# CognitiveAISystems/MAPF-GPT

Hardware: AMD Instinct MI355X
Metric: agent-steps/s (env+obs+GPT fwd) (higher is better)
Workload: dtype f16x3

## Files before the change

mapf_gpt_amd/csrc/gpt_kernels_c256b.h:

```cpp
#pragma once
#include "gpt_kernels_c256p.h"
#include "gpt_kernels_attn_tiles.h"

namespace mgpt {
namespace fastk {

constexpr int kA256oProjSteps = 16;
constexpr int kA256oPeriod = 8 * kA256StepsPerHead + kA256oProjSteps;


template <class T, int NP>
__global__ __launch_bounds__(256) void pack_attn256q_kernel(const float *__restrict__ w_attn, const float *__restrict__ gain,
                                                            const float *__restrict__ w_proj, uint16_t *__restrict__ out,
                                                            float scale_a, float scale_p)
{
    constexpr int C = 256, NH = 8, QKV = NH * kA256StepsPerHead;
    const int64_t gid = (int64_t)blockIdx.x * 256 + threadIdx.x;
    if (gid >= (int64_t)kA256oPeriod * 8 * 64) return;
    const int lane = (int)(gid & 63), ms = (int)((gid >> 6) & 7), G = (int)(gid >> 9);
    const int rho = lane & 15, qk = lane >> 4;
    float v[8];
    if (G < QKV) {
        const int head = G / kA256StepsPerHead, st = G - head * kA256StepsPerHead;
        int which, kb, dim;
        if (st < 4) {
            const int cc = 4 * st + (ms >> 1), ug = ms & 1, rq = rho >> 2;
            kb = cc >> 1; which = cc & 1;
            const int blk = which == 0 ? 2 * (rq & 1) + (rq >> 1) : rq;
            dim = 8 * blk + 4 * ug + (rho & 3);
        } else { which = 2; kb = 4 * (st - 4) + (ms >> 1); dim = 16 * (ms & 1) + rho; }
        const float *row = w_attn + (size_t)(which * C + head * 32 + dim) * C;
#pragma unroll
        for (int e = 0; e < 8; e++) {
            const int col = 32 * kb + 8 * qk + e;
            v[e] = row[col] * gain[col] * scale_a;
        }
    } else {
        const int s = G - QKV, tt = s >> 2, j = s & 3;
        const int cc = 4 * j + (ms >> 1), kb = cc >> 1, fgl = 2 * (cc & 1) + (ms & 1);
        const float *row = w_proj + (size_t)(64 * tt + 16 * fgl + rho) * C;
#pragma unroll
        for (int e = 0; e < 8; e++) {
            const int col = 32 * kb + (e & 3) + 8 * (2 * (qk & 1) + (e >> 2)) + 4 * (qk >> 1);
            v[e] = row[col] * scale_p;
        }
    }
    u32x2 h0, l0, h1, l1;
    split4<T, NP>(v, h0, l0);
    split4<T, NP>(v + 4, h1, l1);
    u32x4 hi, lo;
    hi[0] = h0[0]; hi[1] = h0[1]; hi[2] = h1[0]; hi[3] = h1[1];
    lo[0] = l0[0]; lo[1] = l0[1]; lo[2] = l1[0]; lo[3] = l1[1];
    uint16_t *dst = out + (((size_t)G * 8 + ms) * NP) * 512 + (size_t)lane * 8;
    *reinterpret_cast<u32x4 *>(dst) = hi;
    if (NP == 2) *reinterpret_cast<u32x4 *>(dst + 512) = lo;
}

template <int NP> constexpr int kL0TabHeadBytes = 192 * NP;
template <int NP> constexpr int kL0TabEntryBytes = 8 * kL0TabHeadBytes<NP>;
template <class T, int NP, int STAMPS = 0, bool EMB = false, int TAB = 0>
__global__ __launch_bounds__(512, 2) void attn256q_kernel(float *__restrict__ x, const uint16_t *__restrict__ wstream, float inv_scale,
                                                          float scale_log2e, float inv_proj, unsigned char *__restrict__ spill,
                                                          int n_rows, unsigned long long *stamps = nullptr,
                                                          const unsigned char *__restrict__ tokens = nullptr, const float *__restrict__ etab = nullptr,
                                                          unsigned char *__restrict__ table = nullptr)
{
    static_assert(TAB == 0 || (TAB == 1 && EMB) || (TAB == 2 && !EMB && STAMPS == 0), "table modes");
    constexpr int HB = kL0TabHeadBytes<NP>, ENT = kL0TabEntryBytes<NP>;
    constexpr int C = 256, KS = 16, NH = 8, HS = 32, NW = 8;
    static_assert(NP == 2 || NP == 1, "planes");
    constexpr int MS = 8;
    constexpr int STEP = MS * NP * 1024;
    constexpr int NSLOT = 5;
    constexpr int PW = MS * NP / NW;
    constexpr int KROW = 80, VROW = 528;
    constexpr int NSPILL = 2 * NP;
    constexpr int NYLD = 14 * NP;
    static_assert(PW >= 1, "a wave moves at least one piece per step");
    extern __shared__ __attribute__((aligned(16))) unsigned char smem[];
    const int tid = threadIdx.x, lane = tid & 63;
    const int wave = __builtin_amdgcn_readfirstlane(tid >> 6);
    const int tok0 = wave * 32;
    const unsigned lane16 = (unsigned)lane * 16u;
    const unsigned lds0 = (unsigned)(size_t)smem + lane16;
    const unsigned sK = (unsigned)(size_t)smem + NSLOT * STEP, sV = sK + NP * kT * KROW;
    constexpr int PERIOD = TAB == 2 ? kA256oProjSteps : kA256oPeriod;
    const unsigned char *wbase = reinterpret_cast<const unsigned char *>(wstream) + (size_t)(wave * PW) * 1024 +
                                 (TAB == 2 ? (size_t)(kA256oPeriod - kA256oProjSteps) * STEP : 0);
    unsigned char *sp_wave = spill + ((size_t)blockIdx.x * NW + wave) * (size_t)(14 * NP * 1024);
    const int n_mine = n_rows > (int)blockIdx.x ? (n_rows - 1 - (int)blockIdx.x) / (int)gridDim.x + 1 : 0;
    unsigned long long ts[8] = {0, 0, 0, 0, 0, 0, 0, 0}, t_mark = 0;
    auto phase = [&](int i) {
        if constexpr (STAMPS == 1 || STAMPS == 3) { const unsigned long long t = __builtin_readcyclecounter(); ts[i] += t - t_mark; t_mark = t; }
    };
    auto smark = [&]() { if constexpr (STAMPS == 2) t_mark = __builtin_readcyclecounter(); };
    auto sphase = [&](int i) {
        if constexpr (STAMPS == 2) { const unsigned long long t = __builtin_readcyclecounter(); ts[i] += t - t_mark; t_mark = t; }
    };
    if constexpr (STAMPS != 0) { ts[0] = __builtin_readcyclecounter(); ts[1] = wall_clock64(); t_mark = ts[0]; }
    if (n_mine == 0) return;

    int r_issue = 0;
    int slot_cur = 0, slot_prev = NSLOT - 1;
    unsigned cur_addr = 0, nxt_addr = 0;
    auto issue = [&](int slot) {
        const unsigned char *src = wbase + (size_t)r_issue * STEP;
        unsigned char *dst = smem + (size_t)slot * STEP + (size_t)(wave * PW) * 1024;
#pragma unroll
        for (int i = 0; i < PW; i++) dma_piece(src + lane16, dst, std::integral_constant<int, 0>{}, i);
        r_issue = r_issue + 1 == PERIOD ? 0 : r_issue + 1;
    };
#pragma unroll
    for (int G = 0; G < NSLOT - 1; G++) issue(G);
    auto sync_wait = [&](auto pending_c) {
        vm_wait<decltype(pending_c)::value>();
        __builtin_amdgcn_s_barrier();
    };
    int slot_refill = 0;
    auto sync_issue = [&]() {
        issue(slot_prev);
        const int slot_next = slot_cur + 1 == NSLOT ? 0 : slot_cur + 1;
        cur_addr = lds0 + (unsigned)slot_cur * STEP;
        nxt_addr = lds0 + (unsigned)slot_next * STEP;
        slot_prev = slot_cur;
        slot_cur = slot_next;
    };
    u32x4 wb[2][2][2];
    auto lds_frag = [&](unsigned addr, auto off_c, u32x4 &dst) {
        asm volatile("ds_read_b128 %0, %1 offset:%2" : "=v"(dst) : "v"(addr), "n"(decltype(off_c)::value) : "memory");
    };
    auto lds_pair = [&](unsigned slot_addr, auto ms_c, u32x4 (&dst)[2]) {
        constexpr int ms = decltype(ms_c)::value;
        lds_frag(slot_addr, std::integral_constant<int, ms * NP * 1024>{}, dst[0]);
        if (NP == 2) lds_frag(slot_addr, std::integral_constant<int, (ms * NP + 1) * 1024>{}, dst[1]);
        else dst[1] = dst[0];
    };
    auto chunk_begin = [&](auto c_c, auto next_c) {
        constexpr int c = decltype(c_c)::value;
        asm volatile("s_waitcnt lgkmcnt(0)" ::: "memory");
        __builtin_amdgcn_sched_barrier(0);
        if (c < 3) { lds_pair(cur_addr, std::integral_constant<int, 2 * c + 2>{}, wb[(c + 1) & 1][0]); lds_pair(cur_addr, std::integral_constant<int, 2 * c + 3>{}, wb[(c + 1) & 1][1]); }
        else if (decltype(next_c)::value) { lds_pair(nxt_addr, std::integral_constant<int, 0>{}, wb[0][0]); lds_pair(nxt_addr, std::integral_constant<int, 1>{}, wb[0][1]); }
        __builtin_amdgcn_sched_barrier(0);
    };
    constexpr bool PLACED = true;
    auto chunk_wait = [&]() {
        asm volatile("s_waitcnt lgkmcnt(0)" ::: "memory");
        __builtin_amdgcn_sched_barrier(0);
    };
    auto chunk_read = [&](auto c_c, auto next_c, auto n_c) {
        constexpr int c = decltype(c_c)::value, n = decltype(n_c)::value;
        if constexpr (n < 2 * NP) {
            constexpr int fr = n / NP, pl = n % NP;
            if constexpr (c < 3) lds_frag(cur_addr, std::integral_constant<int, ((2 * c + 2 + fr) * NP + pl) * 1024>{}, wb[(c + 1) & 1][fr][pl]);
            else if constexpr (decltype(next_c)::value) lds_frag(nxt_addr, std::integral_constant<int, (fr * NP + pl) * 1024>{}, wb[0][fr][pl]);
            if constexpr (NP == 1 && (c < 3 || decltype(next_c)::value)) wb[(c + 1) & 1][fr][1] = wb[(c + 1) & 1][fr][0];
            __builtin_amdgcn_sched_barrier(0);
        }
    };
    auto pin6 = [&]() {
#pragma unroll
        for (int n = 0; n < (NP == 2 ? 12 : 4); n++) __builtin_amdgcn_sched_group_barrier(0x008, 1, 0);
        __builtin_amdgcn_sched_barrier(0);
    };
    auto pack_octet = [&](const f32x16 &v, int m, u32x4 (&dst)[2]) {
#pragma unroll
        for (int wd = 0; wd < 4; wd++) {
            unsigned a, b2;
            split2p<T, NP>(v[8 * m + 2 * wd], v[8 * m + 2 * wd + 1], a, b2);
            dst[0][wd] = a; dst[1][wd] = b2;
        }
    };
    auto mm16 = [&](const u32x4 &a, const u32x4 &b2, f32x16 &blk, auto s_c) {
        constexpr int S = decltype(s_c)::value;
        f32x4 c = {blk[4 * S], blk[4 * S + 1], blk[4 * S + 2], blk[4 * S + 3]};
        c = T::mfma16(a, b2, c);
        blk[4 * S] = c[0]; blk[4 * S + 1] = c[1]; blk[4 * S + 2] = c[2]; blk[4 * S + 3] = c[3];
    };
    auto mm16z = [&](const u32x4 &a, const u32x4 &b2, f32x16 &blk, auto s_c) {
        constexpr int S = decltype(s_c)::value;
        f32x4 c = {0.f, 0.f, 0.f, 0.f};
        c = T::mfma16(a, b2, c);
        blk[4 * S] = c[0]; blk[4 * S + 1] = c[1]; blk[4 * S + 2] = c[2]; blk[4 * S + 3] = c[3];
    };
    using I0 = std::integral_constant<int, 0>;
    using I1 = std::integral_constant<int, 1>;
    using I2 = std::integral_constant<int, 2>;
    using I3 = std::integral_constant<int, 3>;
    auto mma4 = [&](const u32x4 (&w0)[2], const u32x4 (&w1)[2], const u32x4 (&x0)[2], const u32x4 (&x1)[2], f32x16 &blk, auto swap_c, auto first_c, auto &&behind) {
        constexpr bool SW = decltype(swap_c)::value, FIRST = decltype(first_c)::value;
        auto one = [&](const u32x4 &w, const u32x4 &xx, auto s_c) {
            if constexpr (SW) mm16(xx, w, blk, s_c); else mm16(w, xx, blk, s_c);
        };
        auto onez = [&](const u32x4 &w, const u32x4 &xx, auto s_c) {
            if constexpr (!FIRST) one(w, xx, s_c);
            else if constexpr (SW) mm16z(xx, w, blk, s_c);
            else mm16z(w, xx, blk, s_c);
        };
        if (NP == 2) {
            onez(w0[1], x0[0], I0{}); behind(I0{}); onez(w1[1], x0[0], I1{}); behind(I1{}); onez(w0[1], x1[0], I2{}); behind(I2{}); onez(w1[1], x1[0], I3{}); behind(I3{});
            one(w0[0], x0[1], I0{}); behind(std::integral_constant<int, 4>{}); one(w1[0], x0[1], I1{}); behind(std::integral_constant<int, 5>{});
            one(w0[0], x1[1], I2{}); one(w1[0], x1[1], I3{});
            one(w0[0], x0[0], I0{}); one(w1[0], x0[0], I1{}); one(w0[0], x1[0], I2{}); one(w1[0], x1[0], I3{});
        } else {
            onez(w0[0], x0[0], I0{}); behind(I0{}); onez(w1[0], x0[0], I1{}); behind(I1{}); onez(w0[0], x1[0], I2{}); behind(I2{}); onez(w1[0], x1[0], I3{});
        }
    };
    auto chunk_body = [&](auto c_c, auto next_c, auto &&mm) {
        if constexpr (PLACED) {
            chunk_wait();
            constexpr bool REFILL = false;
            constexpr int N_REFILL = NP == 2 ? 5 : 2, N_LAST = REFILL ? N_REFILL : 2 * NP - 1, NMF = NP == 2 ? 12 : 4;
            mm([&](auto n_c) {
                constexpr int n = decltype(n_c)::value;
                if constexpr (n < 2 * NP) { __builtin_amdgcn_sched_barrier(0); chunk_read(c_c, next_c, n_c); }
                else if constexpr (REFILL && n == N_REFILL) { __builtin_amdgcn_sched_barrier(0); issue(slot_refill); __builtin_amdgcn_sched_barrier(0); }
            });
#pragma unroll
            for (int n = 0; n < NMF - 1 - N_LAST; n++) __builtin_amdgcn_sched_group_barrier(0x008, 1, 0);
            __builtin_amdgcn_sched_barrier(0);
        } else {
            chunk_begin(c_c, next_c);
            mm([&](auto) {});
            pin6();
        }
    };
    auto fold4 = [&](float v) {
        float a = v, b2 = v;
        asm volatile("s_nop 1\n\tv_permlane16_swap_b32 %0, %1" : "+v"(a), "+v"(b2));
        float c = a + b2, d = c;
        asm volatile("s_nop 1\n\tv_permlane32_swap_b32 %0, %1" : "+v"(c), "+v"(d));
        return c + d;
    };
    auto row_swap = [&](unsigned &a, unsigned &b2) {
        asm volatile("s_nop 1\n\tv_permlane16_swap_b32 %0, %1" : "+v"(a), "+v"(b2));
    };
    auto half_swap = [&](float v, float &lower, float &upper) {
        lower = v; upper = v;
        asm volatile("s_nop 1\n\tv_permlane32_swap_b32 %0, %1" : "+v"(lower), "+v"(upper));
    };
    auto other_half_max = [&](float v) { float a, b2; half_swap(v, a, b2); return fmaxf(a, b2); };
    auto other_half_sum = [&](float v) { float a, b2; half_swap(v, a, b2); return a + b2; };
    constexpr bool QK_UNITS = true;
    const float sc2 = 1.0f;
    const float q_units = scale_log2e * inv_scale, k_units = inv_scale;

    u32x4 xn[KS][2];

    f32x16 qa, ka;
    auto step_pair = [&](auto j_c, auto pending_c, auto &&after_barrier, auto next_c) {
        constexpr int j = decltype(j_c)::value;
        smark();
        sync_wait(pending_c);
        after_barrier();
        sync_issue();
        sphase(2);
        auto chunk = [&](auto c_c) {
            constexpr int c = decltype(c_c)::value;
            constexpr int cc = 4 * j + c, kb = cc >> 1;
            chunk_body(c_c, next_c, [&](auto &&behind) {
                using F = std::integral_constant<bool, (cc < 2)>;
                if constexpr ((cc & 1) == 0) mma4(wb[c & 1][0], wb[c & 1][1], xn[kb], xn[8 + kb], qa, std::false_type{}, F{}, behind);
                else mma4(wb[c & 1][0], wb[c & 1][1], xn[kb], xn[8 + kb], ka, std::false_type{}, F{}, behind);
            });
            asm volatile("" : "+v"(qa), "+v"(ka));
        };
        chunk(I0{}); chunk(I1{}); chunk(I2{}); chunk(I3{});
        sphase(4);
    };
    auto nothing = [&]() {};
    asm volatile("s_waitcnt vmcnt(0)" ::: "memory");
    __builtin_amdgcn_s_barrier();
    nxt_addr = lds0;
    using P4 = std::integral_constant<int, PW * (NSLOT - 3)>;
    using P4S = std::integral_constant<int, PW * (NSLOT - 3) + NSPILL>;

#pragma unroll 1
    for (int k = 0; k < n_mine; k++) {
        const int64_t b = (int64_t)blockIdx.x + (int64_t)k * gridDim.x;
        unsigned char *xw = reinterpret_cast<unsigned char *>(x + (b * kT + tok0) * C);
        unsigned ent0 = 0, ent1 = 0;
        if constexpr (TAB == 2) {
            unsigned l16p = lane16;
            asm volatile("" : "+v"(l16p));
            const unsigned char *tk = tokens + b * kT + tok0;
            const unsigned tt_p = (l16p >> 4) & 15u;
            unsigned id0, id1;
            asm volatile("global_load_ubyte %0, %1, %2" : "=v"(id0) : "v"(tt_p), "s"(tk) : "memory");
            asm volatile("global_load_ubyte %0, %1, %2 offset:16" : "=v"(id1) : "v"(tt_p), "s"(tk) : "memory");
            asm volatile("s_waitcnt vmcnt(0)" : "+v"(id0), "+v"(id1) : : "memory");
            ent0 = ((unsigned)tok0 + tt_p) * 67u + id0;
            ent1 = ((unsigned)tok0 + 16u + tt_p) * 67u + id1;
        } else {
            unsigned l16p = lane16;
            asm volatile("" : "+v"(l16p));
            const unsigned xoff_p = (l16p >> 8) * 1024 + ((l16p >> 4) & 15u) * 32;
            f32x4 xr[32];
            if constexpr (EMB) {
                const unsigned char *tk = tokens + b * kT + tok0;
                const unsigned tt_p = (l16p >> 4) & 15u;
                unsigned id0, id1;
                asm volatile("global_load_ubyte %0, %1, %2" : "=v"(id0) : "v"(tt_p), "s"(tk) : "memory");
                asm volatile("global_load_ubyte %0, %1, %2 offset:16" : "=v"(id1) : "v"(tt_p), "s"(tk) : "memory");
                asm volatile("s_waitcnt vmcnt(0)" : "+v"(id0), "+v"(id1) : : "memory");
                const unsigned q32 = (l16p >> 8) * 32u;
                const unsigned ve0 = (((unsigned)tok0 + tt_p) * 67u + id0) * 1024u + q32;
                const unsigned ve1 = (((unsigned)tok0 + 16u + tt_p) * 67u + id1) * 1024u + q32;
                const unsigned char *eb = reinterpret_cast<const unsigned char *>(etab);
#pragma unroll
                for (int i = 0; i < 32; i++) {
                    if (((i >> 1) & 1) == 0)
                        asm volatile("global_load_dwordx4 %0, %1, %2 offset:%3" : "=v"(xr[2 * (i >> 2) + (i & 1)]) : "v"(ve0), "s"(eb), "n"((i >> 2) * 128 + (i & 1) * 16) : "memory");
                    else
                        asm volatile("global_load_dwordx4 %0, %1, %2 offset:%3" : "=v"(xr[2 * (8 + (i >> 2)) + (i & 1)]) : "v"(ve1), "s"(eb), "n"((i >> 2) * 128 + (i & 1) * 16) : "memory");
                }
            } else {
#pragma unroll
            for (int i = 0; i < 32; i++) {
                const unsigned char *xq = xw + (i >> 2) * 4096;
                asm volatile("global_load_dwordx4 %0, %1, %2 offset:%3" : "=v"(xr[2 * (8 * ((i >> 1) & 1) + (i >> 2)) + (i & 1)]) : "v"(xoff_p), "s"(xq), "n"(((i >> 1) & 1) * 512 + (i & 1) * 16) : "memory");
            }
            }
            asm volatile("s_waitcnt vmcnt(0)" : "+v"(xr[0]), "+v"(xr[1]), "+v"(xr[2]), "+v"(xr[3]), "+v"(xr[4]), "+v"(xr[5]), "+v"(xr[6]), "+v"(xr[7]) : : "memory");
            asm volatile("" : "+v"(xr[8]), "+v"(xr[9]), "+v"(xr[10]), "+v"(xr[11]), "+v"(xr[12]), "+v"(xr[13]), "+v"(xr[14]), "+v"(xr[15]));
            asm volatile("" : "+v"(xr[16]), "+v"(xr[17]), "+v"(xr[18]), "+v"(xr[19]), "+v"(xr[20]), "+v"(xr[21]), "+v"(xr[22]), "+v"(xr[23]));
            asm volatile("" : "+v"(xr[24]), "+v"(xr[25]), "+v"(xr[26]), "+v"(xr[27]), "+v"(xr[28]), "+v"(xr[29]), "+v"(xr[30]), "+v"(xr[31]));
            if constexpr (EMB) {
#pragma unroll
                for (int i = 0; i < 32; i++) {
                    const unsigned char *xq = xw + (i >> 2) * 4096;
                    asm volatile("global_store_dwordx4 %0, %1, %2 offset:%3\n\ts_nop 1" ::"v"(xoff_p), "v"(xr[2 * (8 * ((i >> 1) & 1) + (i >> 2)) + (i & 1)]), "s"(xq), "n"(((i >> 1) & 1) * 512 + (i & 1) * 16) : "memory");
                }
            }
            float rstd[2];
#pragma unroll
            for (int tg = 0; tg < 2; tg++) {
                float sm = 0.f;
#pragma unroll
                for (int i = 0; i < 16; i++) sm += (xr[16 * tg + i][0] + xr[16 * tg + i][1]) + (xr[16 * tg + i][2] + xr[16 * tg + i][3]);
                const float mean = fold4(sm) * (1.0f / (float)C);
                float qv = 0.f;
#pragma unroll
                for (int i = 0; i < 16; i++)
#pragma unroll
                    for (int e = 0; e < 4; e++) { const float d = xr[16 * tg + i][e] - mean; xr[16 * tg + i][e] = d; qv = fmaf(d, d, qv); }
                rstd[tg] = rsqrtf(fold4(qv) * (1.0f / (float)C) + 1e-5f);
            }
#pragma unroll
            for (int ks = 0; ks < KS; ks++) {
                float v0[4], v1[4];
#pragma unroll
                for (int e = 0; e < 4; e++) { v0[e] = xr[2 * ks][e] * rstd[ks >> 3]; v1[e] = xr[2 * ks + 1][e] * rstd[ks >> 3]; }
                u32x2 h0, l0, h1, l1;
                split4p<T, NP>(v0, h0, l0);
                split4p<T, NP>(v1, h1, l1);
                xn[ks][0][0] = h0[0]; xn[ks][0][1] = h0[1]; xn[ks][0][2] = h1[0]; xn[ks][0][3] = h1[1];
                xn[ks][1][0] = l0[0]; xn[ks][1][1] = l0[1]; xn[ks][1][2] = l1[0]; xn[ks][1][3] = l1[1];
                if ((ks & 1) == 1) __builtin_amdgcn_sched_barrier(0);
            }
        }
        if constexpr (TAB != 2) {
            lds_pair(nxt_addr, I0{}, wb[0][0]);
            lds_pair(nxt_addr, I1{}, wb[0][1]);
        }
        phase(2);

        auto head = [&](int hd, auto last_c) {
            constexpr bool LASTH = decltype(last_c)::value;
            unsigned l16 = lane16;
            asm volatile("" : "+v"(l16));
            const unsigned rr = (l16 >> 4) & 31u, hh = l16 >> 9;
            const unsigned kr_addr = sK + rr * KROW + hh * 16;
            const unsigned vr_addr = sV + rr * VROW + hh * 16;
            const unsigned tt = (l16 >> 4) & 15u, qq = l16 >> 8;
            const unsigned kw_addr = sK + ((unsigned)tok0 + tt) * KROW + qq * 16;
            const unsigned vw_addr = sV + tt * VROW + (unsigned)wave * 64 + (qq & 1u) * 16 + (qq >> 1) * 8;
            asm volatile("" : "=v"(qa), "=v"(ka));
            step_pair(I0{}, P4S{}, nothing, std::true_type{});
            step_pair(I1{}, P4S{}, nothing, std::true_type{});
            step_pair(I2{}, P4S{}, nothing, std::true_type{});
            step_pair(I3{}, P4{}, nothing, std::true_type{});
            u32x4 qf[2][2];
            if constexpr (QK_UNITS) {
#pragma unroll
                for (int g = 0; g < 16; g++) { qa[g] *= q_units; ka[g] *= k_units; }
            }
#pragma unroll
            for (int tg = 0; tg < 2; tg++) pack_octet(qa, tg, qf[tg]);
#pragma unroll
            for (int pl = 0; pl < NP; pl++)
#pragma unroll
                for (int wd = 0; wd < 4; wd++) { unsigned a = qf[0][pl][wd], b2 = qf[1][pl][wd]; row_swap(a, b2); qf[0][pl][wd] = a; qf[1][pl][wd] = b2; }
            if (NP == 1) { qf[0][1] = qf[0][0]; qf[1][1] = qf[1][0]; }
            if constexpr (TAB == 1) {
                const unsigned voff = (((unsigned)tok0 + rr) * 67u * ENT) + (unsigned)b * ENT + (unsigned)hd * HB + hh * (32 * NP);
#pragma unroll
                for (int ks = 0; ks < 2; ks++)
#pragma unroll
                    for (int pl = 0; pl < NP; pl++)
                        asm volatile("global_store_dwordx4 %0, %1, %2 offset:%3\n\ts_nop 1" ::"v"(voff), "v"(qf[ks][pl]), "s"(table), "n"((ks * NP + pl) * 16) : "memory");
            }
            {
                u32x4 kp[2][2];
#pragma unroll
                for (int tg = 0; tg < 2; tg++) pack_octet(ka, tg, kp[tg]);
#pragma unroll
                for (int tg = 0; tg < 2; tg++)
#pragma unroll
                    for (int pl = 0; pl < NP; pl++)
                        asm volatile("ds_write_b128 %0, %1 offset:%2" ::"v"(kw_addr), "v"(kp[tg][pl]), "n"(pl * kT * KROW + tg * 16 * KROW) : "memory");
                if constexpr (TAB == 1) {
#pragma unroll
                    for (int tg = 0; tg < 2; tg++) {
                        const unsigned voff = (((unsigned)tok0 + 16u * tg + tt) * 67u * ENT) + (unsigned)b * ENT + (unsigned)hd * HB + 64 * NP + qq * (16 * NP);
#pragma unroll
                        for (int pl = 0; pl < NP; pl++)
                            asm volatile("global_store_dwordx4 %0, %1, %2 offset:%3\n\ts_nop 1" ::"v"(voff), "v"(kp[tg][pl]), "s"(table), "n"(pl * 16) : "memory");
                    }
                }
            }
            f32x16 va;
            auto step_v = [&](auto j_c, auto next_c) {
                constexpr int j = decltype(j_c)::value;
                smark();
                sync_wait(P4{});
                sync_issue();
                sphase(3);
                auto chunk = [&](auto c_c) {
                    constexpr int c = decltype(c_c)::value;
                    constexpr int kb = 4 * j + c;
                    chunk_body(c_c, next_c, [&](auto &&behind) { mma4(wb[c & 1][0], wb[c & 1][1], xn[kb], xn[8 + kb], va, std::true_type{}, std::integral_constant<bool, kb == 0>{}, behind); });
                    asm volatile("" : "+v"(va));
                };
                chunk(I0{}); chunk(I1{}); chunk(I2{}); chunk(I3{});
                sphase(5);
            };
            step_v(I0{}, std::true_type{});
            step_v(I1{}, std::false_type{});
            if constexpr (LASTH) {
#pragma unroll
                for (int hh2 = 0; hh2 < 7; hh2++)
#pragma unroll
                    for (int tg = 0; tg < 2; tg++)
#pragma unroll
                        for (int pl = 0; pl < NP; pl++) {
                            const unsigned char *p = sp_wave + (size_t)hh2 * (size_t)(2 * NP * 1024);
                            asm volatile("global_load_dwordx4 %0, %1, %2 offset:%3" : "=v"(xn[8 * tg + hh2][pl]) : "v"(lane16), "s"(p), "n"((tg * NP + pl) * 1024) : "memory");
                        }
            }
            {
#pragma unroll
                for (int sl = 0; sl < 4; sl++) {
                    u32x2 vp[2];
                    unsigned a0, b0, a1, b1;
                    split2p<T, NP>(va[4 * sl], va[4 * sl + 1], a0, b0);
                    split2p<T, NP>(va[4 * sl + 2], va[4 * sl + 3], a1, b1);
                    vp[0][0] = a0; vp[0][1] = a1; vp[1][0] = b0; vp[1][1] = b1;
#pragma unroll
                    for (int pl = 0; pl < NP; pl++)
                        asm volatile("ds_write_b64 %0, %1 offset:%2" ::"v"(vw_addr), "v"(vp[pl]), "n"(pl * HS * VROW + (sl & 1) * 16 * VROW + (sl >> 1) * 32) : "memory");
                    if constexpr (TAB == 1) {
#pragma unroll
                        for (int i = 0; i < 4; i++) {
                            const unsigned voff = (((unsigned)tok0 + 16u * (sl >> 1) + 4u * qq + i) * 67u * ENT) + (unsigned)b * ENT + (unsigned)hd * HB + 128 * NP +
                                                  (16u * (sl & 1) + tt) * 2u;
#pragma unroll
                            for (int pl = 0; pl < NP; pl++) {
                                if (i & 1) asm volatile("global_store_short_d16_hi %0, %1, %2 offset:%3" ::"v"(voff), "v"(vp[pl][i >> 1]), "s"(table), "n"(pl * 64) : "memory");
                                else asm volatile("global_store_short %0, %1, %2 offset:%3" ::"v"(voff), "v"(vp[pl][i >> 1]), "s"(table), "n"(pl * 64) : "memory");
                            }
                        }
                    }
                }
            }
            if constexpr (TAB == 1) asm volatile("s_waitcnt vmcnt(0)" ::: "memory");
            asm volatile("s_waitcnt lgkmcnt(0)" ::: "memory");
            phase(3);
            __builtin_amdgcn_s_barrier();

            f32x16 o;
            float l_run = 0.f;
            attention_tiles<T, NP, KROW, VROW, HS>(kr_addr, vr_addr, qf, lane, o, l_run);
            lds_pair(nxt_addr, I0{}, wb[0][0]);
            lds_pair(nxt_addr, I1{}, wb[0][1]);
            {
                const float inv = inv_scale / l_run;
#pragma unroll
                for (int g = 0; g < 16; g++) o[g] *= inv;
#pragma unroll
                for (int g = 0; g < 8; g++) { float a = o[g], b2 = o[8 + g]; asm volatile("s_nop 1\n\tv_permlane16_swap_b32 %0, %1" : "+v"(a), "+v"(b2)); o[g] = a; o[8 + g] = b2; }
                if constexpr (LASTH) {
                    pack_octet(o, 0, xn[7]);
                    pack_octet(o, 1, xn[15]);
                } else {
                    u32x4 yp[2][2];
                    pack_octet(o, 0, yp[0]);
                    pack_octet(o, 1, yp[1]);
                    unsigned char *p = sp_wave + (size_t)hd * (size_t)(2 * NP * 1024);
#pragma unroll
                    for (int kk = 0; kk < 2; kk++)
#pragma unroll
                        for (int pl = 0; pl < NP; pl++)
                            asm volatile("global_store_dwordx4 %0, %1, %2 offset:%3\n\ts_nop 1" ::"v"(lane16), "v"(yp[kk][pl]), "s"(p), "n"((kk * NP + pl) * 1024) : "memory");
                }
            }
            phase(4);
        };
        auto head_t = [&](int hd) {
            unsigned l16 = lane16;
            asm volatile("" : "+v"(l16));
            const unsigned rr = (l16 >> 4) & 31u, hh = l16 >> 9;
            const unsigned kr_addr = sK + rr * KROW + hh * 16;
            const unsigned vr_addr = sV + rr * VROW + hh * 16;
            const unsigned tt = (l16 >> 4) & 15u, qq = l16 >> 8;
            const unsigned kw_addr = sK + ((unsigned)tok0 + tt) * KROW + qq * 16;
            const unsigned vt_addr = sV + qq * 8 * VROW + (unsigned)wave * 64 + (((tt >> 2) & 1u) * 8 + ((tt >> 3) & 1u) * 4 + (tt & 3u)) * 2;
            const unsigned hoff = (unsigned)hd * HB;
            const unsigned e0 = ent0 * ENT + hoff, e1 = ent1 * ENT + hoff;
            const unsigned qoff = ((qq & 1u) ? e1 : e0) + hh * (32 * NP);
            u32x4 qf[2][2], kp[2][2], vq[2][2];
#pragma unroll
            for (int ks = 0; ks < 2; ks++)
#pragma unroll
                for (int pl = 0; pl < NP; pl++)
                    asm volatile("global_load_dwordx4 %0, %1, %2 offset:%3" : "=v"(qf[ks][pl]) : "v"(qoff), "s"(table), "n"((ks * NP + pl) * 16) : "memory");
#pragma unroll
            for (int tg = 0; tg < 2; tg++) {
                const unsigned ko = (tg ? e1 : e0) + qq * (16 * NP), vo = (tg ? e1 : e0) + qq * 16;
#pragma unroll
                for (int pl = 0; pl < NP; pl++) {
                    asm volatile("global_load_dwordx4 %0, %1, %2 offset:%3" : "=v"(kp[tg][pl]) : "v"(ko), "s"(table), "n"(64 * NP + pl * 16) : "memory");
                    asm volatile("global_load_dwordx4 %0, %1, %2 offset:%3" : "=v"(vq[tg][pl]) : "v"(vo), "s"(table), "n"(128 * NP + pl * 64) : "memory");
                }
            }
            __builtin_amdgcn_s_barrier();
            if constexpr (NP == 2)
                asm volatile("s_waitcnt vmcnt(0)" : "+v"(qf[0][0]), "+v"(qf[0][1]), "+v"(qf[1][0]), "+v"(qf[1][1]), "+v"(kp[0][0]), "+v"(kp[0][1]), "+v"(kp[1][0]), "+v"(kp[1][1]),
                             "+v"(vq[0][0]), "+v"(vq[0][1]), "+v"(vq[1][0]), "+v"(vq[1][1]) : : "memory");
            else
                asm volatile("s_waitcnt vmcnt(0)" : "+v"(qf[0][0]), "+v"(qf[1][0]), "+v"(kp[0][0]), "+v"(kp[1][0]), "+v"(vq[0][0]), "+v"(vq[1][0]) : : "memory");
            if (NP == 1) { qf[0][1] = qf[0][0]; qf[1][1] = qf[1][0]; }
#pragma unroll
            for (int tg = 0; tg < 2; tg++)
#pragma unroll
                for (int pl = 0; pl < NP; pl++) {
                    asm volatile("ds_write_b128 %0, %1 offset:%2" ::"v"(kw_addr), "v"(kp[tg][pl]), "n"(pl * kT * KROW + tg * 16 * KROW) : "memory");
#pragma unroll
                    for (int j = 0; j < 8; j++) {
                        if (j & 1) asm volatile("ds_write_b16_d16_hi %0, %1 offset:%2" ::"v"(vt_addr), "v"(vq[tg][pl][j >> 1]), "n"(pl * HS * VROW + j * VROW + tg * 32) : "memory");
                        else asm volatile("ds_write_b16 %0, %1 offset:%2" ::"v"(vt_addr), "v"(vq[tg][pl][j >> 1]), "n"(pl * HS * VROW + j * VROW + tg * 32) : "memory");
                    }
                }
            asm volatile("s_waitcnt lgkmcnt(0)" ::: "memory");
            __builtin_amdgcn_s_barrier();
            f32x16 o;
            float l_run = 0.f;
            attention_tiles<T, NP, KROW, VROW, HS>(kr_addr, vr_addr, qf, lane, o, l_run);
            const float inv = inv_scale / l_run;
#pragma unroll
            for (int g = 0; g < 16; g++) o[g] *= inv;
#pragma unroll
            for (int g = 0; g < 8; g++) { float a = o[g], b2 = o[8 + g]; asm volatile("s_nop 1\n\tv_permlane16_swap_b32 %0, %1" : "+v"(a), "+v"(b2)); o[g] = a; o[8 + g] = b2; }
#pragma unroll
            for (int k2 = 0; k2 < 7; k2++)
#pragma unroll
                for (int pl = 0; pl < NP; pl++) { xn[k2][pl] = xn[k2 + 1][pl]; xn[8 + k2][pl] = xn[9 + k2][pl]; }
            pack_octet(o, 0, xn[7]);
            pack_octet(o, 1, xn[15]);
        };
        if constexpr (TAB == 2) {
#pragma unroll 1
            for (int hd = 0; hd < NH; hd++) head_t(hd);
            lds_pair(nxt_addr, I0{}, wb[0][0]);
            lds_pair(nxt_addr, I1{}, wb[0][1]);
        } else {
#pragma unroll 1
            for (int hd = 0; hd < NH - 1; hd++) head(hd, std::false_type{});
            head(NH - 1, std::true_type{});
        }

        auto tail = [&](int t, auto first_c, auto last_c) {
            constexpr bool FIRST = decltype(first_c)::value, LASTT = decltype(last_c)::value;
            asm volatile("" : "=v"(qa), "=v"(ka));
            unsigned l16t = lane16;
            asm volatile("" : "+v"(l16t));
            const unsigned xoff_t = (l16t >> 9) * 1024 + ((l16t >> 4) & 15u) * 32 + ((l16t >> 8) & 1u) * 16;
            const unsigned qq_t = l16t >> 8;
            f32x4 xs[4][2];
            unsigned char *xp = xw + (size_t)t * 8192;
            constexpr int OTHERS = 8;
            auto requests = [&]() {
                if constexpr (TAB == 2) {
                    const unsigned r0 = ent0 * (C * 4) + (unsigned)t * 256 + qq_t * 16, r1 = ent1 * (C * 4) + (unsigned)t * 256 + qq_t * 16;
                    const unsigned char *eb = reinterpret_cast<const unsigned char *>(etab);
#pragma unroll
                    for (int fgl = 0; fgl < 4; fgl++) {
                        asm volatile("global_load_dwordx4 %0, %1, %2 offset:%3" : "=v"(xs[fgl][0]) : "v"(r0), "s"(eb), "n"(fgl * 64) : "memory");
                        asm volatile("global_load_dwordx4 %0, %1, %2 offset:%3" : "=v"(xs[fgl][1]) : "v"(r1), "s"(eb), "n"(fgl * 64) : "memory");
                    }
                    return;
                }
#pragma unroll
                for (int fgl = 0; fgl < 4; fgl++)
#pragma unroll
                    for (int tg = 0; tg < 2; tg++)
                        asm volatile("global_load_dwordx4 %0, %1, %2 offset:%3" : "=v"(xs[fgl][tg]) : "v"(xoff_t), "s"(xp + (fgl >> 1) * 4096), "n"((fgl & 1) * 2048 + tg * 512) : "memory");
            };
            step_pair(I0{}, std::integral_constant<int, 2 * PW + (FIRST ? (TAB == 2 ? 0 : NYLD) : 8)>{}, requests, std::true_type{});
            step_pair(I1{}, std::integral_constant<int, 2 * PW + 8 + OTHERS>{}, nothing, std::true_type{});
            step_pair(I2{}, std::integral_constant<int, 2 * PW + 8 + OTHERS>{}, nothing, std::true_type{});
            step_pair(I3{}, P4{}, nothing, std::integral_constant<bool, !LASTT>{});
            phase(5);
            asm volatile("s_waitcnt vmcnt(%[n])" : "+v"(xs[0][0]), "+v"(xs[0][1]), "+v"(xs[1][0]), "+v"(xs[1][1]), "+v"(xs[2][0]), "+v"(xs[2][1]), "+v"(xs[3][0]), "+v"(xs[3][1])
                         : [n] "n"(4 * PW) : "memory");
#pragma unroll
            for (int fgl = 0; fgl < 4; fgl++)
#pragma unroll
                for (int tg = 0; tg < 2; tg++) {
                    f32x4 v;
#pragma unroll
                    for (int e = 0; e < 4; e++) v[e] = fmaf((fgl < 2 ? qa : ka)[4 * (2 * tg + (fgl & 1)) + e], inv_proj, xs[fgl][tg][e]);
                    asm volatile("global_store_dwordx4 %0, %1, %2 offset:%3\n\ts_nop 1" ::"v"(xoff_t), "v"(v), "s"(xp + (fgl >> 1) * 4096), "n"((fgl & 1) * 2048 + tg * 512) : "memory");
                }
            phase(6);
        };
        {
            asm volatile("s_waitcnt vmcnt(0)" : "+v"(xn[0][0]), "+v"(xn[0][1]), "+v"(xn[1][0]), "+v"(xn[1][1]), "+v"(xn[2][0]), "+v"(xn[2][1]), "+v"(xn[3][0]), "+v"(xn[3][1]),
                         "+v"(xn[4][0]), "+v"(xn[4][1]), "+v"(xn[5][0]), "+v"(xn[5][1]), "+v"(xn[6][0]), "+v"(xn[6][1]) : : "memory");
            asm volatile("" : "+v"(xn[8][0]), "+v"(xn[8][1]), "+v"(xn[9][0]), "+v"(xn[9][1]), "+v"(xn[10][0]), "+v"(xn[10][1]), "+v"(xn[11][0]), "+v"(xn[11][1]),
                         "+v"(xn[12][0]), "+v"(xn[12][1]), "+v"(xn[13][0]), "+v"(xn[13][1]), "+v"(xn[14][0]), "+v"(xn[14][1]));
            asm volatile("" : "+v"(xn[7][0]), "+v"(xn[7][1]), "+v"(xn[15][0]), "+v"(xn[15][1]));
        }
        tail(0, std::true_type{}, std::false_type{});
#pragma unroll 1
        for (int t = 1; t < 3; t++) tail(t, std::false_type{}, std::false_type{});
        tail(3, std::false_type{}, std::true_type{});
    }
    asm volatile("s_waitcnt vmcnt(0)" ::: "memory");
    if constexpr (STAMPS != 0) {
        if (lane == 0 && ((wave == 0 && STAMPS != 3) || (STAMPS == 2 && wave == 4) || (STAMPS == 3 && wave == 4))) {
            ts[7] = wall_clock64();
#pragma unroll
            for (int i = 0; i < 8; i++) stamps[((size_t)blockIdx.x * (STAMPS == 2 ? 2 : 1) + (STAMPS == 2 ? (wave >> 2) : 0)) * 8 + i] = ts[i];
        }
    }
}

}
}
```

Measured before the change: 131,000.

## Synchronise weight-stream ring every two steps with double-slot prefetch

Restructures the LDS weight-streaming ring so that barriers and DMA issues happen once per pair of steps (super-step) rather than every step. The first step of each pair waits, barriers, and issues two slots ahead (cur+3, cur+4). The second step only advances the slot pointers. Prologue prefetch depth and vmcnt pending counts are adjusted to match. This halves the workgroup barriers in the QKV/V/proj GEMM loops, at the cost of a shallower effective prefetch distance and more outstanding loads per sync point.

```diff
diff --git a/mapf_gpt_amd/csrc/gpt_kernels_c256b.h b/mapf_gpt_amd/csrc/gpt_kernels_c256b.h
--- a/mapf_gpt_amd/csrc/gpt_kernels_c256b.h
+++ b/mapf_gpt_amd/csrc/gpt_kernels_c256b.h
@@ -101,7 +101,7 @@
     if (n_mine == 0) return;
 
     int r_issue = 0;
-    int slot_cur = 0, slot_prev = NSLOT - 1;
+    int slot_cur = 0;
     unsigned cur_addr = 0, nxt_addr = 0;
     auto issue = [&](int slot) {
         const unsigned char *src = wbase + (size_t)r_issue * STEP;
@@ -111,20 +111,25 @@
         r_issue = r_issue + 1 == PERIOD ? 0 : r_issue + 1;
     };
 #pragma unroll
-    for (int G = 0; G < NSLOT - 1; G++) issue(G);
-    auto sync_wait = [&](auto pending_c) {
+    for (int G = 0; G < NSLOT - 2; G++) issue(G);
+    int slot_refill = 0;
+    auto sync_top = [&](auto pending_c) {
         vm_wait<decltype(pending_c)::value>();
         __builtin_amdgcn_s_barrier();
-    };
-    int slot_refill = 0;
-    auto sync_issue = [&]() {
-        issue(slot_prev);
-        const int slot_next = slot_cur + 1 == NSLOT ? 0 : slot_cur + 1;
+        const int s1 = slot_cur + 1 == NSLOT ? 0 : slot_cur + 1;
+        issue(slot_cur + 3 >= NSLOT ? slot_cur + 3 - NSLOT : slot_cur + 3);
+        issue(slot_cur + 4 >= NSLOT ? slot_cur + 4 - NSLOT : slot_cur + 4);
         cur_addr = lds0 + (unsigned)slot_cur * STEP;
-        nxt_addr = lds0 + (unsigned)slot_next * STEP;
-        slot_prev = slot_cur;
-        slot_cur = slot_next;
-    };
+        nxt_addr = lds0 + (unsigned)s1 * STEP;
+        slot_cur = s1;
+    };
+    auto step_over = [&]() {
+        const int s1 = slot_cur + 1 == NSLOT ? 0 : slot_cur + 1;
+        cur_addr = lds0 + (unsigned)slot_cur * STEP;
+        nxt_addr = lds0 + (unsigned)s1 * STEP;
+        slot_cur = s1;
+    };
+    using MID = std::integral_constant<int, -1>;
     u32x4 wb[2][2][2];
     auto lds_frag = [&](unsigned addr, auto off_c, u32x4 &dst) {
         asm volatile("ds_read_b128 %0, %1 offset:%2" : "=v"(dst) : "v"(addr), "n"(decltype(off_c)::value) : "memory");
@@ -248,12 +253,12 @@
     u32x4 xn[KS][2];
 
     f32x16 qa, ka;
-    auto step_pair = [&](auto j_c, auto pending_c, auto &&after_barrier, auto next_c) {
+    auto step_pair = [&](auto j_c, auto pending_c, auto &&after_issue, auto next_c) {
         constexpr int j = decltype(j_c)::value;
+        static_assert(((j & 1) == 1) == (decltype(pending_c)::value < 0), "a super-step synchronises at its first step only");
         smark();
-        sync_wait(pending_c);
-        after_barrier();
-        sync_issue();
+        if constexpr ((j & 1) == 0) { sync_top(pending_c); after_issue(); }
+        else step_over();
         sphase(2);
         auto chunk = [&](auto c_c) {
             constexpr int c = decltype(c_c)::value;
@@ -272,8 +277,8 @@
     asm volatile("s_waitcnt vmcnt(0)" ::: "memory");
     __builtin_amdgcn_s_barrier();
     nxt_addr = lds0;
-    using P4 = std::integral_constant<int, PW * (NSLOT - 3)>;
-    using P4S = std::integral_constant<int, PW * (NSLOT - 3) + NSPILL>;
+    using P0 = std::integral_constant<int, 0>;
+    using PS = std::integral_constant<int, NSPILL>;
 
 #pragma unroll 1
     for (int k = 0; k < n_mine; k++) {
@@ -376,10 +381,10 @@
             const unsigned kw_addr = sK + ((unsigned)tok0 + tt) * KROW + qq * 16;
             const unsigned vw_addr = sV + tt * VROW + (unsigned)wave * 64 + (qq & 1u) * 16 + (qq >> 1) * 8;
             asm volatile("" : "=v"(qa), "=v"(ka));
-            step_pair(I0{}, P4S{}, nothing, std::true_type{});
-            step_pair(I1{}, P4S{}, nothing, std::true_type{});
-            step_pair(I2{}, P4S{}, nothing, std::true_type{});
-            step_pair(I3{}, P4{}, nothing, std::true_type{});
+            step_pair(I0{}, PS{}, nothing, std::true_type{});
+            step_pair(I1{}, MID{}, nothing, std::true_type{});
+            step_pair(I2{}, P0{}, nothing, std::true_type{});
+            step_pair(I3{}, MID{}, nothing, std::true_type{});
             u32x4 qf[2][2];
             if constexpr (QK_UNITS) {
 #pragma unroll
@@ -423,8 +428,7 @@
             auto step_v = [&](auto j_c, auto next_c) {
                 constexpr int j = decltype(j_c)::value;
                 smark();
-                sync_wait(P4{});
-                sync_issue();
+                if constexpr (j == 0) sync_top(P0{}); else step_over();
                 sphase(3);
                 auto chunk = [&](auto c_c) {
                     constexpr int c = decltype(c_c)::value;
@@ -606,13 +610,13 @@
                     for (int tg = 0; tg < 2; tg++)
                         asm volatile("global_load_dwordx4 %0, %1, %2 offset:%3" : "=v"(xs[fgl][tg]) : "v"(xoff_t), "s"(xp + (fgl >> 1) * 4096), "n"((fgl & 1) * 2048 + tg * 512) : "memory");
             };
-            step_pair(I0{}, std::integral_constant<int, 2 * PW + (FIRST ? (TAB == 2 ? 0 : NYLD) : 8)>{}, requests, std::true_type{});
-            step_pair(I1{}, std::integral_constant<int, 2 * PW + 8 + OTHERS>{}, nothing, std::true_type{});
-            step_pair(I2{}, std::integral_constant<int, 2 * PW + 8 + OTHERS>{}, nothing, std::true_type{});
-            step_pair(I3{}, P4{}, nothing, std::integral_constant<bool, !LASTT>{});
+            step_pair(I0{}, std::integral_constant<int, FIRST ? 0 : 8>{}, requests, std::true_type{});
+            step_pair(I1{}, MID{}, nothing, std::true_type{});
+            step_pair(I2{}, std::integral_constant<int, OTHERS>{}, nothing, std::true_type{});
+            step_pair(I3{}, MID{}, nothing, std::integral_constant<bool, !LASTT>{});
             phase(5);
             asm volatile("s_waitcnt vmcnt(%[n])" : "+v"(xs[0][0]), "+v"(xs[0][1]), "+v"(xs[1][0]), "+v"(xs[1][1]), "+v"(xs[2][0]), "+v"(xs[2][1]), "+v"(xs[3][0]), "+v"(xs[3][1])
-                         : [n] "n"(4 * PW) : "memory");
+                         : [n] "n"(2 * PW) : "memory");
 #pragma unroll
             for (int fgl = 0; fgl < 4; fgl++)
 #pragma unroll
```

After: 131,400, median of 6. Within noise of the previous version (+0.3%).
